# weibohuang0314/pixel_aware_gyro_aided_klt_feature_tracker

Measured on AMD Instinct MI355X. Metric: tracked features/sec (21x21, 3-lvl, 30 iter), higher is better.
Workload: dtype f32 sampling, f64 normal equations; 1 GPU; cfg1_euroc_752x480: 752x480 pair, 1000 keypoints (1000/GPU), gyro-predicted affine init, h=10, L=3, I=30 (synthetic stand-in for BASELINE configs[1]); mode=shard-weak, features_total=1000, features_active=1000, step_mode=graph

## Files before the change

__graft_entry__.py:

```python
from __future__ import annotations

import os
import subprocess
import sys

ROOT = os.path.dirname(os.path.abspath(__file__))
PKG = os.path.join(ROOT, "pixel_aware_gyro_aided_klt_feature_tracker_amd")
CSRC = os.path.join(PKG, "csrc")
HIP_LIB = os.path.join(PKG, "libpagk_hip.so")
HOST_LIB = os.path.join(PKG, "libpagk_tracker.so")

HIPCC_FLAGS = [
    "--offload-arch=gfx950", "-O3", "-std=c++17", "-fPIC", "-shared",
    "-ffp-contract=off", "-fno-fast-math",
    "-Wall", "-Wno-unused-function",
]


def _newer(target: str, sources: list[str]) -> bool:
    if not os.path.exists(target):
        return False
    t = os.path.getmtime(target)
    return all(os.path.getmtime(s) <= t for s in sources)

# ... 10 lines not shown

RESOURCE_CLAIMS = {
    "k_track_blockILi2ELi25ELi4ELb0ELb0ELb1": (128, 0, 4),
    "k_track_blockILi1ELi25ELi4ELb0ELb0ELb1": (96, 0, 4),
    "k_track_quadILi7ELb1": (128, 44, 4),
    "k_track_blockILi2ELi25ELi4ELb0ELb0ELb0": (128, 20, 4),
    "k_track_blockILi1ELi25ELi4ELb0ELb0ELb0": (128, 6, 4),
    "k_track_quadILi7ELb0": (128, 48, 4),
    "k_track_block_pyrILi2ELi25ELb0": (128, 24, 4),
    "k_track_resume_liveILi2ELi25ELb0": (128, 64, 4),
    "k_track_resumeILi2ELi25ELb0": (128, 64, 4),
    "k_track_resume_liveILi2ELi25ELb1": (128, 48, 4),
    "k_track_resumeILi2ELi25ELb1": (128, 48, 4),
    "k_track_block_pyrILi2ELi25ELb1": (128, 8, 4),
    "k_track_block5ILi2ELi25ELb1": (96, 16, 5),
    "k_rectifyILi1ELb1": (64, 0, 8),
    "k_rectifyILi3ELb1": (64, 0, 8),
    "k_rectifyILi4ELb1": (64, 0, 8),
    "k_match_choose": (64, 0, 8),
    "k_match_compact": (64, 0, 8),
    "k_radius_top2": (64, 0, 8),
    "k_klt_finish": (64, 0, 8),
    "k_pose_prep": (64, 0, 8),
    "k_pose_hyp": (176, 0, 2),
    "k_pose_recover": (112, 0, 4),
    "k_pose_gather": (64, 0, 8),
}


RESOURCE_CLAIMS_ALL_VARIANTS = {
# ... 208 lines not shown
```

include/pagk.h:

```cpp
#ifndef PAGK_H
#define PAGK_H

#include <stddef.h>
#include <stdint.h>

#ifdef __cplusplus
extern "C" {
#endif

#define PAGK_VERSION 303

#define PAGK_MAX_PYRAMIDS 8
#define PAGK_MAX_HALF_PATCH 15

enum {
    PAGK_OK = 0,
    PAGK_E_ARG = -1,
    PAGK_E_HIP = -2,
    PAGK_E_NOMEM = -3,
    PAGK_E_UNSUPPORTED = -4,
    PAGK_E_NODEVICE = -5,
    PAGK_E_NCCL = -6,
    PAGK_E_CAPACITY = -7
};
// ... 83 lines not shown
int pagk_check_launch(pagk_ctx *ctx);
int pagk_set_stream(pagk_ctx *ctx, void *hip_stream);

int pagk_set_kernel(pagk_ctx *ctx, int32_t which);
int pagk_has_variant(int32_t which);
int pagk_last_variant(const pagk_ctx *ctx);

int pagk_last_handover(pagk_ctx *ctx);

int pagk_priority_threshold(pagk_ctx *ctx);

int pagk_prio_hint_threshold(pagk_ctx *ctx);
int pagk_prio_hint_reset(pagk_ctx *ctx);
int pagk_prio_hint_get(pagk_ctx *ctx, int32_t n, int32_t *hints);
int pagk_prio_hint_set(pagk_ctx *ctx, int32_t n, const int32_t *hints);

int pagk_set_concurrency(pagk_ctx *ctx, int32_t streams);

int pagk_last_kernel_ms(pagk_ctx *ctx, float *track_ms, float *pyramid_ms);

int pagk_gyro_predict_device(pagk_ctx *ctx, const pagk_params *params, int32_t width, int32_t height,
                             const float *KRKinv, const float *r3, int32_t n, const float *d_pt_ref_un,
                             float *d_pt_predict_un, float *d_pt_predict, uint8_t *d_status, float *d_affine);
int pagk_gyro_predict_device_rot(pagk_ctx *ctx, const pagk_params *params, int32_t width, int32_t height,
                                 const float *d_rot, int32_t n, const float *d_pt_ref_un, float *d_pt_predict_un,
                                 float *d_pt_predict, uint8_t *d_status, float *d_affine);

int pagk_post_filter(int32_t n, int32_t half_patch, const uint8_t *status_pm,
                     const double *pix_err, const double *dist_pred, const float *pt_pm,
                     const float *pt_pm_un, uint8_t *status_out, float *pt_predict,
// ... 296 lines not shown
```

pixel_aware_gyro_aided_klt_feature_tracker_amd/capi.py:

```python
from __future__ import annotations

import ctypes as C
import os

import numpy as np

PKG_DIR = os.path.dirname(os.path.abspath(__file__))
LIB_PATH = os.environ.get("PAGK_LIB") or os.path.join(PKG_DIR, "libpagk_hip.so")

PAGK_OK = 0
PAGK_E_ARG = -1
PAGK_E_HIP = -2
PAGK_E_NOMEM = -3
PAGK_E_UNSUPPORTED = -4
PAGK_E_NODEVICE = -5
PAGK_E_NCCL = -6
PAGK_E_CAPACITY = -7


class Image(C.Structure):
    _fields_ = [("data", C.c_void_p), ("width", C.c_int32), ("height", C.c_int32), ("step", C.c_int64)]


class Params(C.Structure):
# ... 365 lines not shown
    lib.pagk_ncc_free.argtypes = [vp, _P(Image), _P(Image), i32, i32, vp, vp, vp, vp]
    if hasattr(lib, "pagk_selftest_divide"):
        lib.pagk_selftest_divide.restype = C.c_int
        lib.pagk_selftest_divide.argtypes = [vp, i32, vp, vp, vp, vp, vp, vp]
        lib.pagk_selftest_solve.restype = C.c_int
        lib.pagk_selftest_solve.argtypes = [vp, i32, vp, vp, C.c_uint32, vp, vp, vp, vp]
    if hasattr(lib, "pagk_prio_hint_reset"):
        lib.pagk_prio_hint_threshold.restype = C.c_int
        lib.pagk_prio_hint_threshold.argtypes = [vp]
        lib.pagk_prio_hint_reset.restype = C.c_int
        lib.pagk_prio_hint_reset.argtypes = [vp]
        lib.pagk_prio_hint_get.restype = C.c_int
        lib.pagk_prio_hint_get.argtypes = [vp, i32, vp]
        lib.pagk_prio_hint_set.restype = C.c_int
        lib.pagk_prio_hint_set.argtypes = [vp, i32, vp]
    if hasattr(lib, "pagk_priority_threshold"):
        lib.pagk_priority_threshold.restype = C.c_int
        lib.pagk_priority_threshold.argtypes = [vp]
    if hasattr(lib, "pagk_check_launch"):
        lib.pagk_check_launch.restype = C.c_int
        lib.pagk_check_launch.argtypes = [vp]
    if hasattr(lib, "pagk_selftest_repeat_sum"):
        lib.pagk_selftest_repeat_sum.restype = C.c_int
        lib.pagk_selftest_repeat_sum.argtypes = [vp, i32, vp, i32, vp, vp]
    if hasattr(lib, "pagk_selftest_sample"):
        lib.pagk_selftest_sample.restype = C.c_int
        lib.pagk_selftest_sample.argtypes = [vp, i32, i32, i32, i32, vp, vp]
    lib.pagk_match_features.restype = C.c_int
    lib.pagk_match_features.argtypes = [i32, i32, vp, vp, vp, vp, i32, vp, vp, vp, vp]
    lib.pagk_multi_create.restype = C.c_int
# ... 28 lines not shown
EXPORTED_SYMBOLS = [
    "pagk_version", "pagk_strerror", "pagk_last_error", "pagk_params_default", "pagk_inv_log_max_dist",
    "pagk_create", "pagk_destroy", "pagk_track", "pagk_track_pyr", "pagk_frame_upload", "pagk_frame_upload_pinned",
    "pagk_frame_set_device", "pagk_frame_download_level", "pagk_track_device", "pagk_track_device_fused", "pagk_sync",
    "pagk_set_stream", "pagk_set_kernel", "pagk_last_variant", "pagk_set_concurrency", "pagk_last_handover", "pagk_last_kernel_ms", "pagk_post_filter", "pagk_gyro_predict_device",
    "pagk_gyro_predict_device_rot",
    "pagk_geometry_scores_device", "pagk_geometry_scores", "pagk_geometry_select", "pagk_geometry_validation",
    "pagk_graph_begin", "pagk_graph_end", "pagk_graph_launch", "pagk_graph_destroy",
    "pagk_near_neighbors_device", "pagk_find_near_neighbors", "pagk_ncc_free", "pagk_match_features",
    "pagk_multi_create", "pagk_multi_unique_id", "pagk_multi_create_rank", "pagk_multi_destroy", "pagk_multi_world",
    "pagk_multi_local", "pagk_multi_ctx", "pagk_multi_last_error", "pagk_shard_range", "pagk_shard_layout",
    "pagk_multi_allgather", "pagk_track_sharded", "pagk_selftest_divide", "pagk_selftest_solve",
    "pagk_selftest_repeat_sum", "pagk_check_launch", "pagk_track_device_batch", "pagk_frame_set_device_batch", "pagk_priority_threshold",
    "pagk_multi_comm_count", "pagk_has_variant",
    "pagk_prio_hint_threshold", "pagk_prio_hint_reset", "pagk_prio_hint_get", "pagk_prio_hint_set",
    "pagk_fit_params_default", "pagk_geometry_fit_device", "pagk_geometry_fit", "pagk_geometry_validation_device",
    "pagk_geometry_validation_fit", "pagk_selftest_fit_samples",
    "pagk_pose_params_default", "pagk_pose_params_check", "pagk_pose_2d2d_device", "pagk_pose_from_matches_device",
    "pagk_pose_2d2d",
    "pagk_post_filter_device", "pagk_gyro_predict_device_live", "pagk_frame_handover_device", "pagk_frame_handover",
    "pagk_detect_params_default", "pagk_detect_corners_device", "pagk_detect_corners",
    "pagk_frame_handover_detect_device", "pagk_frame_handover_detect", "pagk_selftest_corner_response",
    "pagk_fast_params_default", "pagk_fast_params_check", "pagk_detect_fast_bounds", "pagk_detect_fast_device",
    "pagk_detect_fast", "pagk_frame_handover_fast_device", "pagk_frame_handover_fast", "pagk_selftest_fast_cells",
    "pagk_rectify_params_default", "pagk_rectify_params_check", "pagk_rectify_set_maps", "pagk_frame_rectify_device",
    "pagk_frame_rectify_pinned", "pagk_rectify", "pagk_undistort_maps",
    "pagk_orb_params_default", "pagk_orb_params_check", "pagk_orb_pattern_check", "pagk_orb_set_pattern",
    "pagk_orb_describe_device", "pagk_orb_describe", "pagk_orb_match_device", "pagk_orb_match",
    "pagk_selftest_sample",
    "pagk_lk_params_default", "pagk_lk_params_check", "pagk_lk_levels", "pagk_lk_pyramid_device", "pagk_lk_track_device",
# ... 939 lines not shown
        return int(self.lib.pagk_prio_hint_threshold(self.h))

    def prio_hint_reset(self):
        if hasattr(self.lib, "pagk_prio_hint_reset"):
            self._check(self.lib.pagk_prio_hint_reset(self.h), "pagk_prio_hint_reset")

    def prio_hint_get(self, n: int) -> np.ndarray:
        out = np.zeros(max(n, 0), np.int32)
        self._check(self.lib.pagk_prio_hint_get(self.h, n, out.ctypes.data_as(C.c_void_p)), "pagk_prio_hint_get")
        return out

    def prio_hint_set(self, hints) -> None:
        h = np.ascontiguousarray(hints, np.int32)
        self._check(self.lib.pagk_prio_hint_set(self.h, int(h.shape[0]), h.ctypes.data_as(C.c_void_p)), "pagk_prio_hint_set")

    def last_variant(self) -> int:
        return int(self.lib.pagk_last_variant(self.h))

    def last_handover(self) -> int:
        rc = int(self.lib.pagk_last_handover(self.h))
        if rc < 0:
            self._check(rc, "pagk_last_handover")
        return rc

    def set_concurrency(self, streams: int):
        self._check(self.lib.pagk_set_concurrency(self.h, streams), "pagk_set_concurrency")

    def last_kernel_ms(self):
        t, p = C.c_float(0), C.c_float(0)
        self._check(self.lib.pagk_last_kernel_ms(self.h, C.byref(t), C.byref(p)), "pagk_last_kernel_ms")
# ... 128 lines not shown
```

pixel_aware_gyro_aided_klt_feature_tracker_amd/csrc/pagk_device.h:

```cpp
#pragma once
#include <hip/hip_runtime.h>
#include <stdint.h>

namespace pagk {

constexpr int kMaxLevels = 8;

struct DevLevel {
    const uint32_t *quad;
    int cols, rows;
    float fcols, frows;
    float fcols_m1, frows_m1;
};

__device__ __forceinline__ int ld_agent(const int *p) { return __hip_atomic_load(p, __ATOMIC_RELAXED, __HIP_MEMORY_SCOPE_AGENT); }
__device__ __forceinline__ void st_agent(int *p, int v) { __hip_atomic_store(p, v, __ATOMIC_RELAXED, __HIP_MEMORY_SCOPE_AGENT); }

struct SuspState {
    int level;
    int iter;
    float dx, dy, dg, db, lastCost;
    int iters;
};

// ... 46 lines not shown
    int half, iterations;
    int prio_k;
    unsigned long long *prio_stats;
    const int *prio_kbuf;
    const int *prio_hint_in;
    int *prio_hint_out;
    int prio_hint_t;
    int has_gyro, illum, use_affine, penalty, calc_ncc;
    uint32_t solver;
    float lam_invlog;
    float lam_invlog_alpha;
    float alpha;
    double win_size_inv;
    int distort_on;
    float fx, fy, cx, cy, fx_inv, fy_inv, k1, k2, p1, p2, k3;
};

__device__ __forceinline__ DevLevel pin_level(const DevLevel &src) { return src; }

struct Coord {
    int i;
    float f;
    float omf;
};

template <bool CLAMP>
__device__ __forceinline__ Coord prep_coord(float x, float fmax, float fmax_m1)
{
    if (CLAMP) {
        x = fmaxf(x, 0.0f);
// ... 667 lines not shown
```

pixel_aware_gyro_aided_klt_feature_tracker_amd/csrc/pagk_hip.hip:

```cpp
#include <hip/hip_runtime.h>

#include <algorithm>
#include <array>
#include <cmath>
#include <cstdio>
#include <cstdlib>
#include <cstring>
#include <new>
#include <utility>
#include <vector>

#include "../../include/pagk.h"
#include "pagk_kernels.h"
#include "pagk_associate_kernel.h"
#include "pagk_pose_kernel.h"
#include "pagk_layout.h"
#include "pagk_select.h"
#include "pagk_prio_env.h"

using namespace pagk;

namespace {

constexpr int kSlots = 6;
constexpr int kUserSlots = 4;

struct DevBuf {
    void *ptr = nullptr;
    size_t bytes = 0;
    void *host = nullptr;
    bool mirrored = false;
};

// ... 27 lines not shown
        FAST,
        RECT_ENTRIES,
        RECT_STAGE,
        ORB_PATTERN,
        ORB_BLUR,
        ORB_KEYS,
        LK_PYR,
        LK_PYR_LAST = LK_PYR + kSlots - 1,
        ASSOC,
        POSE,
        POSEIO,
        QUAD_WS,
        SUSP,
        LV,
        PRIO_HINT,
        kBufs
    };
    DevBuf buf[kBufs];
    int fit_n = 0, fit_iters = 0;
    int pose_n = 0, pose_iters = 0;
    int rect_w = 0, rect_h = 0, rect_wp = 0;
    bool orb_pattern_set = false;
    struct LkPyr { int w = 0, h = 0, top = -1; } lk_pyr[kSlots];
    void *queue = nullptr;
    int quad_capacity[PAGK_MAX_HALF_PATCH + 1] = {};
    int rows_capacity[PAGK_MAX_HALF_PATCH + 1] = {};
    int rows_waves_cap = 0;
    int *susp_count_dev = nullptr;
    struct BatchDesc {
        void *host = nullptr, *dev = nullptr;
// ... 34 lines not shown
    std::vector<BatchDesc> graph_batch[kGraphs];
    std::vector<GraphSeg> cap_segs;
    hipEvent_t ev_trk[2] = {}, ev_pyr[2] = {};
    bool trk_timed = false, pyr_timed = false;
    int kernel = 0;
    bool last_handover = false;
    int concurrency = 1;
    int last_variant = -1;
    int mfma_min_features = 0x7fffffff;
    int wave_min_features = 6000;
    int quad_min_features = 7000;
    int block5_min_features = 2500;
    int prio_k = 4;
    unsigned long long *prio_stats = nullptr;
    int prio_hint_t = kPrioHintDefault;
    bool block5_window = true;
    int levels_min_features = 6000;
    int levels_shift = 0;
    bool levels_shared = false;
    bool unfused_pyramid = false;
    char err[256] = {0};
};

namespace {

#define HIPCHK(ctx, call)                                                                              \
    do {                                                                                               \
        hipError_t e_ = (call);                                                                        \
        if (e_ != hipSuccess) {                                                                        \
            snprintf((ctx)->err, sizeof((ctx)->err), "%s:%d %s -> %s", __FILE__, __LINE__, #call,     \
// ... 116 lines not shown
    Layout<N> lay_;
    void *base_ = nullptr, *own_ = nullptr;
    bool pending_ = false;
};

int capture_split(pagk_ctx *ctx)
{
    hipGraph_t g = nullptr;
    HIPCHK(ctx, hipStreamEndCapture(ctx->stream, &g));
    if (g) {
        pagk_ctx::GraphSeg seg;
        hipError_t e = hipGraphInstantiate(&seg.ex, g, nullptr, nullptr, 0);
        if (e != hipSuccess) {
            (void)hipGraphDestroy(g);
            ctx->capturing = false;
            snprintf(ctx->err, sizeof(ctx->err), "hipGraphInstantiate (segment) -> %s", hipGetErrorString(e));
            return PAGK_E_HIP;
        }
        seg.g = g;
        ctx->cap_segs.push_back(seg);
    }
    hipError_t e = hipStreamBeginCapture(ctx->stream, hipStreamCaptureModeThreadLocal);
    if (e != hipSuccess) {
        ctx->capturing = false;
        snprintf(ctx->err, sizeof(ctx->err), "hipStreamBeginCapture (next segment) -> %s", hipGetErrorString(e));
        return PAGK_E_HIP;
    }
    return PAGK_OK;
}
void destroy_segs(std::vector<pagk_ctx::GraphSeg> &v)
{
    for (auto &sg : v) {
        if (sg.ex) (void)hipGraphExecDestroy(sg.ex);
        if (sg.g) (void)hipGraphDestroy(sg.g);
    }
    v.clear();
}

int batch_desc_alloc(pagk_ctx *ctx, pagk_ctx::BatchDesc &d)
// ... 70 lines not shown
    for (int l = 0; l < L; l++) {
        s.u8[l] = lay.at<uint8_t>(s.block.ptr, l);
        s.quad[l] = lay.at<uint32_t>(s.block.ptr, L + l);
    }
    s.w = lw[0];
    s.h = lh[0];
    s.L = L;
    return PAGK_OK;
}

int slot_reserve(pagk_ctx *ctx, FrameSlot &s, int w, int h, int L)
{
    int lw[kMaxLevels], lh[kMaxLevels];
    int rc = level_dims(w, h, L, lw, lh);
    return rc ? rc : slot_alloc(ctx, s, lw, lh, L, NOT_IN_CAPTURE);
}

int make_pyr_args(const FrameSlot &s, const uint8_t *src0, int64_t pitch0, int wrap0, PyrArgs *out)
{
    int lw[kMaxLevels], lh[kMaxLevels];
    level_dims(s.w, s.h, s.L, lw, lh);
    PyrArgs pa;
    memset(&pa, 0, sizeof pa);
    pa.src = src0;
    pa.pitch = pitch0;
    pa.wrap0 = wrap0;
    pa.n_levels = s.L;
    int nb = 0;
    for (int l = 0; l < 4; l++) {
        pa.first_block[l] = nb;
// ... 21 lines not shown
}

int slot_build(pagk_ctx *ctx, FrameSlot &s, const uint8_t *src0, int64_t pitch0, int wrap0)
{
    s.pad0 = wrap0 ? 0 : 2;
    s.img0 = src0, s.pitch0 = pitch0;
    int lw[kMaxLevels], lh[kMaxLevels];
    level_dims(s.w, s.h, s.L, lw, lh);
    dim3 blk(32, 8);
    if (ctx->ev_pyr[0] && !in_capture(ctx)) HIPCHK(ctx, hipEventRecord(ctx->ev_pyr[0], ctx->stream));
    bool all_even = true;
    for (int l = 0; l + 1 < s.L; l++) all_even = all_even && !(lw[l] & 1) && !(lh[l] & 1);
    if (s.L <= 4 && !ctx->unfused_pyramid && all_even) {
        PyrArgs pa;
        const int nb = make_pyr_args(s, src0, pitch0, wrap0, &pa);
        hipLaunchKernelGGL(k_pyramid_fused, dim3(nb), dim3(256), 0, ctx->stream, pa);
        HIPCHK(ctx, hipGetLastError());
        if (ctx->ev_pyr[1] && !in_capture(ctx)) HIPCHK(ctx, hipEventRecord(ctx->ev_pyr[1], ctx->stream));
        if (!in_capture(ctx)) ctx->pyr_timed = true;
        s.wrap0 = wrap0;
        s.valid = true;
        return PAGK_OK;
    }
    const uint8_t *src = src0;
    int64_t pitch = pitch0;
    for (int l = 0; l < s.L; l++) {
        if (l > 0) {
            dim3 grd((lw[l] + 31) / 32, (lh[l] + 7) / 8);
            if (!(lw[l - 1] & 1) && !(lh[l - 1] & 1))
                hipLaunchKernelGGL(k_pyr_down, grd, blk, 0, ctx->stream, src, pitch, lw[l], lh[l], s.u8[l]);
            else
                hipLaunchKernelGGL(k_pyr_down_linear, grd, blk, 0, ctx->stream, src, pitch, lw[l - 1], lh[l - 1], lw[l],
// ... 307 lines not shown
    }
    const bool five = lean && k.block5 && select_block5(n, ctx->block5_min_features, ctx->block5_window, ctx->cus);
    const TrackFn kern = five ? k.block5 : k.block[lean];
    if (lds > 48 * 1024) {
        static thread_local bool configured[PAGK_MAX_HALF_PATCH + 1][2][16] = {};
        bool &done = configured[a.half][lean][ctx->device & 15];
        if (!done) {
            HIPCHK(ctx, hipFuncSetAttribute(reinterpret_cast<const void *>(kern), hipFuncAttributeMaxDynamicSharedMemorySize, (int)lds));
            done = true;
        }
    }
    HIPCHK(ctx, launch(kern, n, kBlock, lds, ctx->stream, a));
    return PAGK_OK;
}

int prio_hint_attach(pagk_ctx *ctx, int n, TrackArgs *a)
{
    DevBuf &hb = ctx->buf[pagk_ctx::PRIO_HINT];
    const size_t need = (size_t)n * sizeof(int32_t);
    if (need > hb.bytes) {
        if (in_capture(ctx)) return PAGK_OK;
        for (int k = 0; k < pagk_ctx::kGraphs; k++)
            if (ctx->graph_execs[k]) return PAGK_OK;
        if (int rc = reserve(ctx, hb, need, NOT_IN_CAPTURE_NOR_UNDER_GRAPH, "the priority hints", kLargestLaunchFirst)) return rc;
        HIPCHK(ctx, hipMemsetAsync(hb.ptr, 0, hb.bytes, ctx->stream));
    }
    a->prio_hint_in = a->prio_hint_out = static_cast<int *>(hb.ptr);
    return PAGK_OK;
}

int prio_hint_clear(pagk_ctx *ctx)
{
    DevBuf &hb = ctx->buf[pagk_ctx::PRIO_HINT];
    if (hb.ptr) HIPCHK(ctx, hipMemsetAsync(hb.ptr, 0, hb.bytes, ctx->stream));
    return PAGK_OK;
}

int launch_track(pagk_ctx *ctx, const pagk_params *p, const FrameSlot &sr, const FrameSlot &sc, int n,
                 const float *d_pt_ref, const float *d_pt_init, const float *d_affine, const uint8_t *d_status,
                 const pagk_outputs *o, const PyrArgs *pyr = nullptr, int pyr_blocks = 0, bool *pyr_done = nullptr,
                 bool hinted = true)
{
    if (pyr_done) *pyr_done = false;
    TrackArgs a;
    memset(&a, 0, sizeof a);
    a.n_levels = p->pyramids;
    for (int l = 0; l < p->pyramids; l++) {
        fill_level(a.l1[l], sr, l);
        fill_level(a.l2[l], sc, l);
// ... 27 lines not shown
        const bool lean = !a.penalty && a.solver == 0;
        const TrackKernels &k = track_kernels_of(a.half);
        const int variant = ctx->last_variant = select_variant(select_in(ctx, p, n));
        int rc = PAGK_OK;
        hipError_t e = hipSuccess;
        switch (variant) {
            case 1: e = launch(k_track_thread, (n + 63) / 64, 64, 0, ctx->stream, a); break;
            case 2: e = launch(k.mfma[lean], n, 128, track_mfma_lds_bytes(a.half), ctx->stream, a); break;
            case 3: e = launch(k.wave[lean], n, 64, track_wave_lds_bytes(a.half), ctx->stream, a); break;
            case 4: e = launch(k.relaxed, n, kBlock, track_block_lds_bytes(a.half), ctx->stream, a); break;
            case 5:
            case 7: rc = launch_quad(ctx, p, k, lean, variant == 7, n, a); break;
            case 6: rc = launch_rows(ctx, k, n, a); break;
            default:
                if (hinted && (rc = prio_hint_attach(ctx, n, &a))) break;
                rc = launch_block(ctx, k, lean, n, a, pyr, pyr_blocks, pyr_done);
                break;
        }
        if (rc) return rc;
        HIPCHK(ctx, e);
        HIPCHK(ctx, hipGetLastError());
    }
    if (ctx->ev_trk[1] && !in_capture(ctx)) HIPCHK(ctx, hipEventRecord(ctx->ev_trk[1], ctx->stream));
    if (!in_capture(ctx)) ctx->trk_timed = true;
    return PAGK_OK;
}

struct FeatPtrs {
    float *pt_ref, *pt_init, *affine;
    uint8_t *status_in;
    pagk_outputs out;
// ... 182 lines not shown
    if (getenv("PAGK_QUAD_MIN")) ctx->quad_min_features = atoi(getenv("PAGK_QUAD_MIN"));
    if (getenv("PAGK_BLOCK5_MIN")) ctx->block5_min_features = atoi(getenv("PAGK_BLOCK5_MIN")), ctx->block5_window = false;
    if (getenv("PAGK_LEVELS_MIN")) ctx->levels_min_features = atoi(getenv("PAGK_LEVELS_MIN"));
    if (getenv("PAGK_PRIO_K") && strcmp(getenv("PAGK_PRIO_K"), "auto") == 0) {
        struct { unsigned long long st[2]; int k, pad; } seed = {{3500ull, 1000ull}, ctx->prio_k, 0};
        if (hipMalloc(reinterpret_cast<void **>(&ctx->prio_stats), sizeof seed) != hipSuccess ||
            hipMemcpy(ctx->prio_stats, &seed, sizeof seed, hipMemcpyHostToDevice) != hipSuccess) {
            if (ctx->prio_stats) (void)hipFree(ctx->prio_stats);
            ctx->prio_stats = nullptr;
            (void)hipGetLastError();
        }
    } else if (getenv("PAGK_PRIO_K")) {
        ctx->prio_k = atoi(getenv("PAGK_PRIO_K")) < 0 ? 0 : atoi(getenv("PAGK_PRIO_K"));
    }
    if (getenv("PAGK_PRIO_HINT")) ctx->prio_hint_t = prio_hint_parse(getenv("PAGK_PRIO_HINT"), ctx->prio_hint_t);
    if (getenv("PAGK_LEVELS_XCD_SHIFT")) ctx->levels_shift = atoi(getenv("PAGK_LEVELS_XCD_SHIFT")) & 7;
    if (getenv("PAGK_LEVELS_SHARED")) ctx->levels_shared = atoi(getenv("PAGK_LEVELS_SHARED")) != 0;
    if (getenv("PAGK_QUAD_BUDGET")) ctx->quad_budget = atoi(getenv("PAGK_QUAD_BUDGET"));
    if (getenv("PAGK_ROWS_WAVES")) ctx->rows_waves_cap = atoi(getenv("PAGK_ROWS_WAVES"));
    if (getenv("PAGK_FINISHER_WGS")) ctx->finisher_wgs = atoi(getenv("PAGK_FINISHER_WGS"));
    if (getenv("PAGK_SUSPEND_LONE")) ctx->susp_lone = atoi(getenv("PAGK_SUSPEND_LONE"));
    if (getenv("PAGK_FINISHER_POLLS")) ctx->finisher_polls = atoi(getenv("PAGK_FINISHER_POLLS"));
    if (getenv("PAGK_LEVEL_POLLS")) ctx->level_polls = atoi(getenv("PAGK_LEVEL_POLLS"));
    if (hipStreamCreateWithFlags(&ctx->aux_stream, hipStreamNonBlocking) != hipSuccess ||
        hipEventCreateWithFlags(&ctx->ev_fork, hipEventDisableTiming) != hipSuccess ||
        hipEventCreateWithFlags(&ctx->ev_join, hipEventDisableTiming) != hipSuccess ||
        hipEventCreateWithFlags(&ctx->ev_batch, hipEventDisableTiming) != hipSuccess) {
        pagk_destroy(ctx);
        return PAGK_E_HIP;
    }
// ... 99 lines not shown
    if (!ctx) return PAGK_E_ARG;
    HIPCHK(ctx, hipSetDevice(ctx->device));
    return prio_hint_clear(ctx);
}

int pagk_prio_hint_get(pagk_ctx *ctx, int32_t n, int32_t *hints)
{
    if (!ctx || n < 0 || (n > 0 && !hints)) return PAGK_E_ARG;
    NOT_WHILE_CAPTURING(ctx, "pagk_prio_hint_get");
    HIPCHK(ctx, hipSetDevice(ctx->device));
    const DevBuf &hb = ctx->buf[pagk_ctx::PRIO_HINT];
    const size_t have = hb.bytes / sizeof(int32_t) < (size_t)n ? hb.bytes / sizeof(int32_t) : (size_t)n;
    memset(hints, 0, (size_t)n * sizeof(int32_t));
    if (have) HIPCHK(ctx, hipMemcpyAsync(hints, hb.ptr, have * sizeof(int32_t), hipMemcpyDeviceToHost, ctx->stream));
    HIPCHK(ctx, hipStreamSynchronize(ctx->stream));
    return PAGK_OK;
}

int pagk_prio_hint_set(pagk_ctx *ctx, int32_t n, const int32_t *hints)
{
    if (!ctx || n < 0 || (n > 0 && !hints)) return PAGK_E_ARG;
    NOT_WHILE_CAPTURING(ctx, "pagk_prio_hint_set");
    HIPCHK(ctx, hipSetDevice(ctx->device));
    DevBuf &hb = ctx->buf[pagk_ctx::PRIO_HINT];
    if (int rc = reserve(ctx, hb, (size_t)n * sizeof(int32_t), NOT_IN_CAPTURE_NOR_UNDER_GRAPH, "the priority hints", kLargestLaunchFirst)) return rc;
    if (int rc = prio_hint_clear(ctx)) return rc;
    if (n) HIPCHK(ctx, hipMemcpyAsync(hb.ptr, hints, (size_t)n * sizeof(int32_t), hipMemcpyHostToDevice, ctx->stream));
    HIPCHK(ctx, hipStreamSynchronize(ctx->stream));
    return PAGK_OK;
}

int pagk_check_launch(pagk_ctx *ctx)
{
    if (!ctx) return PAGK_E_ARG;
    return lv_check(ctx);
}

int pagk_set_concurrency(pagk_ctx *ctx, int32_t streams)
{
    if (!ctx || streams < 1 || streams > 64) return PAGK_E_ARG;
    ctx->concurrency = streams;
    return PAGK_OK;
}

int pagk_sync(pagk_ctx *ctx)
{
    if (!ctx) return PAGK_E_ARG;
    NOT_WHILE_CAPTURING(ctx, "pagk_sync");
    HIPCHK(ctx, hipStreamSynchronize(ctx->stream));
    return lv_check(ctx);
}

int pagk_last_kernel_ms(pagk_ctx *ctx, float *track_ms, float *pyramid_ms)
{
    if (!ctx) return PAGK_E_ARG;
    NOT_WHILE_CAPTURING(ctx, "pagk_last_kernel_ms");
    if (track_ms) {
        *track_ms = 0.0f;
        if (ctx->trk_timed) {
            HIPCHK(ctx, hipEventSynchronize(ctx->ev_trk[1]));
            HIPCHK(ctx, hipEventElapsedTime(track_ms, ctx->ev_trk[0], ctx->ev_trk[1]));
        }
    }
    if (pyramid_ms) {
// ... 1789 lines not shown
        for (auto &d : ctx->cap_batch)
            if (int ar = batch_desc_alloc(ctx, d)) {
                batch_desc_free(ctx->cap_batch);
                return ar;
            }
    }
    HIPCHK(ctx, hipStreamBeginCapture(ctx->stream, hipStreamCaptureModeThreadLocal));
    ctx->capturing = true;
    return PAGK_OK;
}

int pagk_graph_end(pagk_ctx *ctx, int32_t *graph_id)
{
    if (!ctx || !ctx->capturing || !graph_id) return PAGK_E_ARG;
    ctx->capturing = false;
    hipGraph_t g = nullptr;
    HIPCHK(ctx, hipStreamEndCapture(ctx->stream, &g));
    int id = -1;
    for (int k = 0; k < pagk_ctx::kGraphs; k++)
        if (!ctx->graph_execs[k]) {
            id = k;
            break;
        }
    if (id < 0 || !g) {
        if (g) (void)hipGraphDestroy(g);
        destroy_segs(ctx->cap_segs);
        batch_desc_free(ctx->cap_batch);
        snprintf(ctx->err, sizeof(ctx->err), id < 0 ? "all %d graph slots are in use" : "capture produced no graph (%d)", pagk_ctx::kGraphs);
        return PAGK_E_ARG;
    }
    hipGraphExec_t ex = nullptr;
    hipError_t e = hipGraphInstantiate(&ex, g, nullptr, nullptr, 0);
    if (e != hipSuccess) {
        (void)hipGraphDestroy(g);
        destroy_segs(ctx->cap_segs);
        batch_desc_free(ctx->cap_batch);
        snprintf(ctx->err, sizeof(ctx->err), "hipGraphInstantiate -> %s", hipGetErrorString(e));
        return PAGK_E_HIP;
    }
    ctx->graphs[id] = g;
    ctx->graph_execs[id] = ex;
    ctx->pre_segs[id] = std::move(ctx->cap_segs);
    ctx->cap_segs.clear();
    batch_desc_free(ctx->graph_batch[id]);
    ctx->graph_batch[id] = std::move(ctx->cap_batch);
    ctx->cap_batch.clear();
    ctx->cap_batch_used = 0;
    *graph_id = id;
    return PAGK_OK;
}

int pagk_graph_launch(pagk_ctx *ctx, int32_t graph_id)
{
    if (!ctx || ctx->capturing || graph_id < 0 || graph_id >= pagk_ctx::kGraphs || !ctx->graph_execs[graph_id]) return PAGK_E_ARG;
    for (pagk_ctx::GraphSeg &sg : ctx->pre_segs[graph_id]) {
        if (sg.kind == pagk_ctx::GraphSeg::GRAPH) {
            HIPCHK(ctx, hipGraphLaunch(sg.ex, ctx->stream));
        } else if (sg.kind == pagk_ctx::GraphSeg::FINISHER) {
            HIPCHK(ctx, hipEventRecord(ctx->ev_fork, ctx->stream));
            HIPCHK(ctx, hipStreamWaitEvent(ctx->aux_stream, ctx->ev_fork, 0));
            void *kargs[] = {&sg.args};
            HIPCHK(ctx, hipLaunchKernel(sg.fn, dim3(sg.grid), dim3(kBlock), kargs, sg.lds, ctx->aux_stream));
            HIPCHK(ctx, hipEventRecord(ctx->ev_join, ctx->aux_stream));
        } else {
            HIPCHK(ctx, hipStreamWaitEvent(ctx->stream, ctx->ev_join, 0));
        }
    }
    HIPCHK(ctx, hipGraphLaunch(ctx->graph_execs[graph_id], ctx->stream));
    return PAGK_OK;
}

int pagk_graph_destroy(pagk_ctx *ctx, int32_t graph_id)
{
    if (!ctx || graph_id < 0 || graph_id >= pagk_ctx::kGraphs || !ctx->graph_execs[graph_id]) return PAGK_E_ARG;
    HIPCHK(ctx, hipStreamSynchronize(ctx->stream));
    if (ctx->aux_stream) HIPCHK(ctx, hipStreamSynchronize(ctx->aux_stream));
    (void)hipGraphExecDestroy(ctx->graph_execs[graph_id]);
    (void)hipGraphDestroy(ctx->graphs[graph_id]);
    destroy_segs(ctx->pre_segs[graph_id]);
    batch_desc_free(ctx->graph_batch[graph_id]);
    ctx->graph_execs[graph_id] = nullptr;
    ctx->graphs[graph_id] = nullptr;
    return lv_check(ctx);
}

int pagk_geometry_scores_device(pagk_ctx *ctx, const double *H21, const double *H12, const double *F21,
                                int32_t n, const float *d_pts1, const float *d_pts2, float sigma,
                                uint8_t *d_inliers_H, uint8_t *d_inliers_F, float *d_scores)
{
    if (!ctx || !H21 || !H12 || !F21 || n < 0 || !d_scores) return PAGK_E_ARG;
    if (n > 0 && (!d_pts1 || !d_pts2 || !d_inliers_H || !d_inliers_F)) return PAGK_E_ARG;
    HIPCHK(ctx, hipSetDevice(ctx->device));
    ScoreArgs a;
    memset(&a, 0, sizeof a);
    for (int k = 0; k < 9; k++) a.H21[k] = H21[k], a.H12[k] = H12[k], a.F21[k] = F21[k];
    a.pts1 = d_pts1, a.pts2 = d_pts2, a.n = n, a.sigma = sigma;
    a.inl_H = d_inliers_H, a.inl_F = d_inliers_F, a.scores = d_scores;
// ... 952 lines not shown
```

pixel_aware_gyro_aided_klt_feature_tracker_amd/csrc/pagk_kernels.h:

```cpp
#pragma once
#include <type_traits>
#include "pagk_device.h"
#include "pagk_chain_asm.h"
#include "pagk_prio.h"

namespace pagk {

__global__ void k_pyr_down(const uint8_t *__restrict__ src, int64_t pitch, int dw, int dh,
                           uint8_t *__restrict__ dst)
{
    int x = blockIdx.x * blockDim.x + threadIdx.x;
    int y = blockIdx.y * blockDim.y + threadIdx.y;
    if (x >= dw || y >= dh) return;
    const uint8_t *r0 = src + (int64_t)(2 * y) * pitch + 2 * x;
    const uint8_t *r1 = r0 + pitch;
    dst[(int64_t)y * dw + x] = (uint8_t)((r0[0] + r0[1] + r1[0] + r1[1] + 2) >> 2);
}

__global__ void k_pyr_down_linear(const uint8_t *__restrict__ src, int64_t pitch, int w, int h, int dw, int dh,
                                  double scale_x, double scale_y, uint8_t *__restrict__ dst)
{
    const int dx = blockIdx.x * blockDim.x + threadIdx.x;
    const int dy = blockIdx.y * blockDim.y + threadIdx.y;
    if (dx >= dw || dy >= dh) return;
// ... 92 lines not shown
}

__device__ __forceinline__ void pyr_block(const PyrArgs &a, int b, int tid)
{
    if (b < a.first_block[1]) {
        pyr_emit<0>(a, (b - a.first_block[0]) * 256 + tid);
    } else if (b < a.first_block[2]) {
        pyr_emit<1>(a, (b - a.first_block[1]) * 256 + tid);
    } else if (b < a.first_block[3]) {
        pyr_emit<2>(a, (b - a.first_block[2]) * 256 + tid);
    } else if (b < a.first_block[4]) {
        pyr_emit<3>(a, (b - a.first_block[3]) * 256 + tid);
    }
}

__global__ void __launch_bounds__(256) k_pyramid_fused(PyrArgs a)
{
    pyr_block(a, (int)blockIdx.x, (int)threadIdx.x);
}

struct PyrBatchEntry {
    PyrArgs a;
    int block_base, pad_;
};
__global__ void __launch_bounds__(256) k_pyramid_fused_batch(const PyrBatchEntry *__restrict__ frames, int k)
{
    int f = 0;
    for (int j = 1; j < k; j++) f = (int)blockIdx.x >= frames[j].block_base ? j : f;
    pyr_block(frames[f].a, (int)blockIdx.x - frames[f].block_base, (int)threadIdx.x);
}

struct PredictArgs {
    int n, width, height;
// ... 838 lines not shown
        for (int k = 0; k < 6; k++) dbgp[(size_t)i * 16 + k] = st[k];
        dbgp[(size_t)i * 16 + 6] = (unsigned long long)iters;
        dbgp[(size_t)i * 16 + 7] = rt_begin;
        for (int k = 8; k < 11; k++) dbgp[(size_t)i * 16 + k] = st[k];
        dbgp[(size_t)i * 16 + 11] = __builtin_amdgcn_s_memrealtime();
        dbgp[(size_t)i * 16 + 12] = st[12];
        dbgp[(size_t)i * 16 + 13] = st[13];
    }
#endif
#undef STAMP
}

template <int NR, int TAIL, int WAVES = 4, bool MFMA = false, bool RELAXED = false, bool LEAN = false>
__global__ void __launch_bounds__(WAVES * 64, 4) k_track_block(TrackArgs a)
{
    track_block_body<NR, TAIL, WAVES, MFMA, RELAXED, LEAN>(a, (int)blockIdx.x);
}

template <int NR, int TAIL, bool LEAN = false>
__global__ void __launch_bounds__(256, 5) k_track_block5(TrackArgs a)
{
    track_block_body<NR, TAIL, 4, false, false, LEAN, false>(a, (int)blockIdx.x);
}

__device__ __forceinline__ SuspState load_susp_state(const TrackArgs &a, int i)
{
    const int *p = reinterpret_cast<const int *>(&a.susp_state[i]);
    SuspState st;
    st.level = ld_agent(p + 0), st.iter = ld_agent(p + 1);
    st.dx = __int_as_float(ld_agent(p + 2)), st.dy = __int_as_float(ld_agent(p + 3));
    st.dg = __int_as_float(ld_agent(p + 4)), st.db = __int_as_float(ld_agent(p + 5));
    st.lastCost = __int_as_float(ld_agent(p + 6)), st.iters = ld_agent(p + 7);
    return st;
}

template <int NR, int TAIL, bool LEAN = false>
__global__ void __launch_bounds__(256, 4) k_track_resume_live(TrackArgs a)
// ... 39 lines not shown
        if (entry <= 0) continue;
        const int i = entry - 1;
        const SuspState st = load_susp_state(a, i);
        track_block_body<NR, TAIL, 4, false, false, LEAN>(a, i, &st);
        __syncthreads();
    }
}

template <int NR, int TAIL, bool LEAN = false>
__global__ void __launch_bounds__(256, 4) k_track_block_pyr(TrackArgs a, PyrArgs pa)
{
    if ((int)blockIdx.x >= a.n) {
        pyr_block(pa, (int)blockIdx.x - a.n, (int)threadIdx.x);
        return;
    }
    track_block_body<NR, TAIL, 4, false, false, LEAN>(a, (int)blockIdx.x);
}

}

#include "pagk_wave_kernel.h"
#include "pagk_quad_kernel.h"
#ifdef PAGK_ALL_VARIANTS
#include "pagk_rows_kernel.h"
#endif
#include "pagk_score_kernel.h"
#include "pagk_fit_kernel.h"
#include "pagk_handover_kernel.h"
#include "pagk_detect_kernel.h"
#include "pagk_fast_kernel.h"
#include "pagk_rectify_kernel.h"
// ... 5 lines not shown
```

pixel_aware_gyro_aided_klt_feature_tracker_amd/csrc/pagk_prio.h:

```cpp
#pragma once

#ifndef PAGK_PRIO_MODE
#define PAGK_PRIO_MODE 1
#endif

namespace pagk {
__device__ __forceinline__ void prio_account(const TrackArgs &a, int i, int iters, int levels)
{
    if (a.prio_stats && (i & 7) == 0) {
        __hip_atomic_fetch_add(a.prio_stats + 0, (unsigned long long)iters, __ATOMIC_RELAXED, __HIP_MEMORY_SCOPE_AGENT);
        __hip_atomic_fetch_add(a.prio_stats + 1, (unsigned long long)levels, __ATOMIC_RELAXED, __HIP_MEMORY_SCOPE_AGENT);
        if ((i & 63) == 0 && iters <= 4 * levels) {
            const unsigned long long it = __hip_atomic_load(a.prio_stats + 0, __ATOMIC_RELAXED, __HIP_MEMORY_SCOPE_AGENT);
            const unsigned long long lv = __hip_atomic_load(a.prio_stats + 1, __ATOMIC_RELAXED, __HIP_MEMORY_SCOPE_AGENT);
            if (lv > 0) {
                int k = (int)ceilf((float)it / (float)lv);
                k = k < 3 ? 3 : (k > 12 ? 12 : k);
                __hip_atomic_store(const_cast<int *>(a.prio_kbuf), k, __ATOMIC_RELAXED, __HIP_MEMORY_SCOPE_AGENT);
            }
        }
    }
}

constexpr int kPrioBoost = 1 << 20;
__device__ __forceinline__ void prio_hint_store(const TrackArgs &a, int i, int iters)
{
    if (a.prio_hint_out) a.prio_hint_out[i] = iters;
}
}
#if PAGK_PRIO_MODE == 0
#define PAGK_PRIO_DECL(hinted)
#define PAGK_PRIO_TIER
#define PAGK_PRIO_RESET
#define PRIO(n) __builtin_amdgcn_s_setprio(n);
#define PAGK_PRIO_N_CHAIN 3
#define PAGK_PRIO_N_SAMP 2
#define PAGK_PRIO_N_COST 1
#define PAGK_PRIO_N_REST 0
#else
#define PAGK_PRIO_DECL(hinted)                                                                                       \
    int tier_now = 0;                                                                                                \
    const int prio_kv = !kPrioByWork ? 0 : (a.prio_kbuf ? __builtin_amdgcn_readfirstlane(*a.prio_kbuf) : a.prio_k);  \
// ... 32 lines not shown
```

Baseline: 12.69 million features/s.

## Dispatch features longest-first using iteration hints sorted inside pyramid kernel

Adds a counting sort of per-feature iteration hints from the previous frame. It runs as an extra lead block in the fused pyramid kernel and writes a dispatch-order array. The track kernels then map blockIdx through that array, so features expected to need the most iterations are scheduled first, which is meant to cut tail imbalance at the end of the grid. In exchange it adds an indirection load per block, an extra block and LDS in the pyramid launch, and fairly intricate host-side state tracking for graph capture and replay, including a device sync when a graph is replayed on a different stream.

```diff
diff --git a/__graft_entry__.py b/__graft_entry__.py
--- a/__graft_entry__.py
+++ b/__graft_entry__.py
@@ -48,6 +48,7 @@
     "k_track_resumeILi2ELi25ELb1": (128, 48, 4),
     "k_track_block_pyrILi2ELi25ELb1": (128, 8, 4),
     "k_track_block5ILi2ELi25ELb1": (96, 16, 5),
+    "k_pyramid_fused": (64, 0, 8),
     "k_rectifyILi1ELb1": (64, 0, 8),
     "k_rectifyILi3ELb1": (64, 0, 8),
     "k_rectifyILi4ELb1": (64, 0, 8),
diff --git a/include/pagk.h b/include/pagk.h
--- a/include/pagk.h
+++ b/include/pagk.h
@@ -121,6 +121,9 @@
 int pagk_prio_hint_reset(pagk_ctx *ctx);
 int pagk_prio_hint_get(pagk_ctx *ctx, int32_t n, int32_t *hints);
 int pagk_prio_hint_set(pagk_ctx *ctx, int32_t n, const int32_t *hints);
+
+int pagk_dispatch_order_enabled(pagk_ctx *ctx);
+int pagk_dispatch_order_get(pagk_ctx *ctx, int32_t n, int32_t *order, int32_t *in_force);
 
 int pagk_set_concurrency(pagk_ctx *ctx, int32_t streams);
 
diff --git a/pixel_aware_gyro_aided_klt_feature_tracker_amd/capi.py b/pixel_aware_gyro_aided_klt_feature_tracker_amd/capi.py
--- a/pixel_aware_gyro_aided_klt_feature_tracker_amd/capi.py
+++ b/pixel_aware_gyro_aided_klt_feature_tracker_amd/capi.py
@@ -403,6 +403,11 @@
         lib.pagk_prio_hint_get.argtypes = [vp, i32, vp]
         lib.pagk_prio_hint_set.restype = C.c_int
         lib.pagk_prio_hint_set.argtypes = [vp, i32, vp]
+    if hasattr(lib, "pagk_dispatch_order_get"):
+        lib.pagk_dispatch_order_enabled.restype = C.c_int
+        lib.pagk_dispatch_order_enabled.argtypes = [vp]
+        lib.pagk_dispatch_order_get.restype = C.c_int
+        lib.pagk_dispatch_order_get.argtypes = [vp, i32, vp, vp]
     if hasattr(lib, "pagk_priority_threshold"):
         lib.pagk_priority_threshold.restype = C.c_int
         lib.pagk_priority_threshold.argtypes = [vp]
@@ -461,6 +466,7 @@
     "pagk_selftest_repeat_sum", "pagk_check_launch", "pagk_track_device_batch", "pagk_frame_set_device_batch", "pagk_priority_threshold",
     "pagk_multi_comm_count", "pagk_has_variant",
     "pagk_prio_hint_threshold", "pagk_prio_hint_reset", "pagk_prio_hint_get", "pagk_prio_hint_set",
+    "pagk_dispatch_order_enabled", "pagk_dispatch_order_get",
     "pagk_fit_params_default", "pagk_geometry_fit_device", "pagk_geometry_fit", "pagk_geometry_validation_device",
     "pagk_geometry_validation_fit", "pagk_selftest_fit_samples",
     "pagk_pose_params_default", "pagk_pose_params_check", "pagk_pose_2d2d_device", "pagk_pose_from_matches_device",
@@ -1430,6 +1436,16 @@
         h = np.ascontiguousarray(hints, np.int32)
         self._check(self.lib.pagk_prio_hint_set(self.h, int(h.shape[0]), h.ctypes.data_as(C.c_void_p)), "pagk_prio_hint_set")
 
+    def dispatch_order_enabled(self) -> bool:
+        return bool(self.lib.pagk_dispatch_order_enabled(self.h))
+
+    def dispatch_order_get(self, n: int):
+        out = np.zeros(max(n, 0), np.int32)
+        in_force = C.c_int32(0)
+        self._check(self.lib.pagk_dispatch_order_get(self.h, n, out.ctypes.data_as(C.c_void_p), C.byref(in_force)),
+                    "pagk_dispatch_order_get")
+        return out, bool(in_force.value)
+
     def last_variant(self) -> int:
         return int(self.lib.pagk_last_variant(self.h))
 
diff --git a/pixel_aware_gyro_aided_klt_feature_tracker_amd/csrc/pagk_device.h b/pixel_aware_gyro_aided_klt_feature_tracker_amd/csrc/pagk_device.h
--- a/pixel_aware_gyro_aided_klt_feature_tracker_amd/csrc/pagk_device.h
+++ b/pixel_aware_gyro_aided_klt_feature_tracker_amd/csrc/pagk_device.h
@@ -84,6 +84,7 @@
     double win_size_inv;
     int distort_on;
     float fx, fy, cx, cy, fx_inv, fy_inv, k1, k2, p1, p2, k3;
+    const int *order;
 };
 
 __device__ __forceinline__ DevLevel pin_level(const DevLevel &src) { return src; }
diff --git a/pixel_aware_gyro_aided_klt_feature_tracker_amd/csrc/pagk_hip.hip b/pixel_aware_gyro_aided_klt_feature_tracker_amd/csrc/pagk_hip.hip
--- a/pixel_aware_gyro_aided_klt_feature_tracker_amd/csrc/pagk_hip.hip
+++ b/pixel_aware_gyro_aided_klt_feature_tracker_amd/csrc/pagk_hip.hip
@@ -17,6 +17,7 @@
 #include "pagk_layout.h"
 #include "pagk_select.h"
 #include "pagk_prio_env.h"
+#include "pagk_order.h"
 
 using namespace pagk;
 
@@ -74,6 +75,7 @@
         SUSP,
         LV,
         PRIO_HINT,
+        DISPATCH_ORDER,
         kBufs
     };
     DevBuf buf[kBufs];
@@ -138,6 +140,8 @@
     int prio_k = 4;
     unsigned long long *prio_stats = nullptr;
     int prio_hint_t = kPrioHintDefault;
+    bool graph_order[kGraphs] = {};
+    OrderState order;
     bool block5_window = true;
     int levels_min_features = 6000;
     int levels_shift = 0;
@@ -284,6 +288,7 @@
         if (e != hipSuccess) {
             (void)hipGraphDestroy(g);
             ctx->capturing = false;
+            (void)ctx->order.capture_ended();
             snprintf(ctx->err, sizeof(ctx->err), "hipGraphInstantiate (segment) -> %s", hipGetErrorString(e));
             return PAGK_E_HIP;
         }
@@ -293,6 +298,7 @@
     hipError_t e = hipStreamBeginCapture(ctx->stream, hipStreamCaptureModeThreadLocal);
     if (e != hipSuccess) {
         ctx->capturing = false;
+        (void)ctx->order.capture_ended();
         snprintf(ctx->err, sizeof(ctx->err), "hipStreamBeginCapture (next segment) -> %s", hipGetErrorString(e));
         return PAGK_E_HIP;
     }
@@ -393,6 +399,15 @@
     int lw[kMaxLevels], lh[kMaxLevels];
     int rc = level_dims(w, h, L, lw, lh);
     return rc ? rc : slot_alloc(ctx, s, lw, lh, L, NOT_IN_CAPTURE);
+}
+
+int capture_kind(pagk_ctx *ctx) { return ctx->capturing ? 1 : (in_capture(ctx) ? 2 : 0); }
+
+OrderArgs order_build_args(pagk_ctx *ctx)
+{
+    const DevBuf &hb = ctx->buf[pagk_ctx::PRIO_HINT], &ob = ctx->buf[pagk_ctx::DISPATCH_ORDER];
+    const int n = ctx->order.build_n(ctx->stream, ctx->cus, (long long)(hb.bytes / sizeof(int32_t)), (long long)(ob.bytes / sizeof(int32_t)), capture_kind(ctx));
+    return {static_cast<const int *>(hb.ptr), static_cast<int *>(ob.ptr), n};
 }
 
 int make_pyr_args(const FrameSlot &s, const uint8_t *src0, int64_t pitch0, int wrap0, PyrArgs *out)
@@ -444,8 +459,10 @@
     if (s.L <= 4 && !ctx->unfused_pyramid && all_even) {
         PyrArgs pa;
         const int nb = make_pyr_args(s, src0, pitch0, wrap0, &pa);
-        hipLaunchKernelGGL(k_pyramid_fused, dim3(nb), dim3(256), 0, ctx->stream, pa);
+        const OrderArgs oa = order_build_args(ctx);
+        hipLaunchKernelGGL(k_pyramid_fused, dim3(nb + (oa.n > 0 ? 1 : 0)), dim3(256), order_lds_bytes(oa.n), ctx->stream, pa, oa);
         HIPCHK(ctx, hipGetLastError());
+        if (oa.n > 0) ctx->order.built(oa.n, ctx->stream, capture_kind(ctx));
         if (ctx->ev_pyr[1] && !in_capture(ctx)) HIPCHK(ctx, hipEventRecord(ctx->ev_pyr[1], ctx->stream));
         if (!in_capture(ctx)) ctx->pyr_timed = true;
         s.wrap0 = wrap0;
@@ -783,10 +800,21 @@
     return PAGK_OK;
 }
 
+int order_reserve(pagk_ctx *ctx, int n)
+{
+    DevBuf &ob = ctx->buf[pagk_ctx::DISPATCH_ORDER];
+    if (!ctx->order.on || !order_serves(n, ctx->cus) || (size_t)n * sizeof(int32_t) <= ob.bytes || in_capture(ctx)) return PAGK_OK;
+    for (int k = 0; k < pagk_ctx::kGraphs; k++)
+        if (ctx->graph_execs[k]) return PAGK_OK;
+    ctx->order.array_replaced();
+    return reserve(ctx, ob, (size_t)n * sizeof(int32_t), NOT_IN_CAPTURE_NOR_UNDER_GRAPH, "the dispatch order", kLargestLaunchFirst);
+}
+
 int prio_hint_attach(pagk_ctx *ctx, int n, TrackArgs *a)
 {
     DevBuf &hb = ctx->buf[pagk_ctx::PRIO_HINT];
     const size_t need = (size_t)n * sizeof(int32_t);
+    if (int rc = order_reserve(ctx, n)) return rc;
     if (need > hb.bytes) {
         if (in_capture(ctx)) return PAGK_OK;
         for (int k = 0; k < pagk_ctx::kGraphs; k++)
@@ -802,6 +830,7 @@
 {
     DevBuf &hb = ctx->buf[pagk_ctx::PRIO_HINT];
     if (hb.ptr) HIPCHK(ctx, hipMemsetAsync(hb.ptr, 0, hb.bytes, ctx->stream));
+    ctx->order.hints_cleared();
     return PAGK_OK;
 }
 
@@ -859,7 +888,11 @@
             case 6: rc = launch_rows(ctx, k, n, a); break;
             default:
                 if (hinted && (rc = prio_hint_attach(ctx, n, &a))) break;
+                if (a.prio_hint_in && ctx->order.usable(n, ctx->stream, ctx->cus, capture_kind(ctx)) &&
+                    ctx->buf[pagk_ctx::DISPATCH_ORDER].bytes >= (size_t)n * sizeof(int32_t))
+                    a.order = static_cast<const int *>(ctx->buf[pagk_ctx::DISPATCH_ORDER].ptr);
                 rc = launch_block(ctx, k, lean, n, a, pyr, pyr_blocks, pyr_done);
+                if (!rc && hinted) ctx->order.launched(a.prio_hint_out ? n : 0, ctx->stream, a.order != nullptr, capture_kind(ctx));
                 break;
         }
         if (rc) return rc;
@@ -1072,6 +1105,7 @@
         ctx->prio_k = atoi(getenv("PAGK_PRIO_K")) < 0 ? 0 : atoi(getenv("PAGK_PRIO_K"));
     }
     if (getenv("PAGK_PRIO_HINT")) ctx->prio_hint_t = prio_hint_parse(getenv("PAGK_PRIO_HINT"), ctx->prio_hint_t);
+    if (getenv("PAGK_DISPATCH_ORDER")) ctx->order.on = atoi(getenv("PAGK_DISPATCH_ORDER")) != 0;
     if (getenv("PAGK_LEVELS_XCD_SHIFT")) ctx->levels_shift = atoi(getenv("PAGK_LEVELS_XCD_SHIFT")) & 7;
     if (getenv("PAGK_LEVELS_SHARED")) ctx->levels_shared = atoi(getenv("PAGK_LEVELS_SHARED")) != 0;
     if (getenv("PAGK_QUAD_BUDGET")) ctx->quad_budget = atoi(getenv("PAGK_QUAD_BUDGET"));
@@ -1201,6 +1235,24 @@
     memset(hints, 0, (size_t)n * sizeof(int32_t));
     if (have) HIPCHK(ctx, hipMemcpyAsync(hints, hb.ptr, have * sizeof(int32_t), hipMemcpyDeviceToHost, ctx->stream));
     HIPCHK(ctx, hipStreamSynchronize(ctx->stream));
+    ctx->order.stream_idle(ctx->stream);
+    return PAGK_OK;
+}
+
+int pagk_dispatch_order_enabled(pagk_ctx *ctx) { return ctx ? (ctx->order.on ? 1 : 0) : PAGK_E_ARG; }
+
+int pagk_dispatch_order_get(pagk_ctx *ctx, int32_t n, int32_t *order, int32_t *in_force)
+{
+    if (!ctx || n < 0 || (n > 0 && !order)) return PAGK_E_ARG;
+    NOT_WHILE_CAPTURING(ctx, "pagk_dispatch_order_get");
+    HIPCHK(ctx, hipSetDevice(ctx->device));
+    const DevBuf &ob = ctx->buf[pagk_ctx::DISPATCH_ORDER];
+    const size_t have = ob.bytes / sizeof(int32_t) < (size_t)n ? ob.bytes / sizeof(int32_t) : (size_t)n;
+    for (int32_t i = 0; i < n; i++) order[i] = i;
+    if (have) HIPCHK(ctx, hipMemcpyAsync(order, ob.ptr, have * sizeof(int32_t), hipMemcpyDeviceToHost, ctx->stream));
+    HIPCHK(ctx, hipStreamSynchronize(ctx->stream));
+    ctx->order.stream_idle(ctx->stream);
+    if (in_force) *in_force = (have == (size_t)n && ctx->order.usable(n, ctx->stream, ctx->cus, 0)) ? 1 : 0;
     return PAGK_OK;
 }
 
@@ -1214,6 +1266,9 @@
     if (int rc = prio_hint_clear(ctx)) return rc;
     if (n) HIPCHK(ctx, hipMemcpyAsync(hb.ptr, hints, (size_t)n * sizeof(int32_t), hipMemcpyHostToDevice, ctx->stream));
     HIPCHK(ctx, hipStreamSynchronize(ctx->stream));
+    if (int rc = order_reserve(ctx, n)) return rc;
+    ctx->order.stream_idle(ctx->stream);
+    ctx->order.hints_set(n);
     return PAGK_OK;
 }
 
@@ -1235,6 +1290,7 @@
     if (!ctx) return PAGK_E_ARG;
     NOT_WHILE_CAPTURING(ctx, "pagk_sync");
     HIPCHK(ctx, hipStreamSynchronize(ctx->stream));
+    ctx->order.stream_idle(ctx->stream);
     return lv_check(ctx);
 }
 
@@ -3054,6 +3110,7 @@
 {
     if (!ctx || !ctx->capturing || !graph_id) return PAGK_E_ARG;
     ctx->capturing = false;
+    const bool carries_order = ctx->order.capture_ended();
     hipGraph_t g = nullptr;
     HIPCHK(ctx, hipStreamEndCapture(ctx->stream, &g));
     int id = -1;
@@ -3080,6 +3137,7 @@
     }
     ctx->graphs[id] = g;
     ctx->graph_execs[id] = ex;
+    ctx->graph_order[id] = carries_order;
     ctx->pre_segs[id] = std::move(ctx->cap_segs);
     ctx->cap_segs.clear();
     batch_desc_free(ctx->graph_batch[id]);
@@ -3093,6 +3151,7 @@
 int pagk_graph_launch(pagk_ctx *ctx, int32_t graph_id)
 {
     if (!ctx || ctx->capturing || graph_id < 0 || graph_id >= pagk_ctx::kGraphs || !ctx->graph_execs[graph_id]) return PAGK_E_ARG;
+    if (ctx->graph_order[graph_id] && ctx->order.replay(ctx->stream)) HIPCHK(ctx, hipDeviceSynchronize());
     for (pagk_ctx::GraphSeg &sg : ctx->pre_segs[graph_id]) {
         if (sg.kind == pagk_ctx::GraphSeg::GRAPH) {
             HIPCHK(ctx, hipGraphLaunch(sg.ex, ctx->stream));
@@ -3121,6 +3180,11 @@
     batch_desc_free(ctx->graph_batch[graph_id]);
     ctx->graph_execs[graph_id] = nullptr;
     ctx->graphs[graph_id] = nullptr;
+    ctx->graph_order[graph_id] = false;
+    ctx->order.stream_idle(ctx->stream);
+    bool alive = false;
+    for (int k = 0; k < pagk_ctx::kGraphs; k++) alive = alive || ctx->graph_execs[k];
+    if (!alive) ctx->order.graphs_gone();
     return lv_check(ctx);
 }
 
diff --git a/pixel_aware_gyro_aided_klt_feature_tracker_amd/csrc/pagk_kernels.h b/pixel_aware_gyro_aided_klt_feature_tracker_amd/csrc/pagk_kernels.h
--- a/pixel_aware_gyro_aided_klt_feature_tracker_amd/csrc/pagk_kernels.h
+++ b/pixel_aware_gyro_aided_klt_feature_tracker_amd/csrc/pagk_kernels.h
@@ -3,6 +3,7 @@
 #include "pagk_device.h"
 #include "pagk_chain_asm.h"
 #include "pagk_prio.h"
+#include "pagk_order.h"
 
 namespace pagk {
 
@@ -130,9 +131,83 @@
     }
 }
 
-__global__ void __launch_bounds__(256) k_pyramid_fused(PyrArgs a)
-{
-    pyr_block(a, (int)blockIdx.x, (int)threadIdx.x);
+struct OrderArgs {
+    const int *hints;
+    int *order;
+    int n;
+};
+
+__device__ __forceinline__ void order_block(const OrderArgs &o, int tid)
+{
+    extern __shared__ __attribute__((aligned(16))) unsigned char order_lds[];
+    int (*s_at)[kOrderClasses] = reinterpret_cast<int (*)[kOrderClasses]>(order_lds);
+    uint8_t *s_class = order_lds + 4 * kOrderClasses * sizeof(int);
+    const int n = o.n < kOrderMaxN ? o.n : kOrderMaxN;
+    const int wave = tid >> 6, lane = tid & 63;
+    const int quarter = ((n + 255) >> 8) << 6;
+    const int lo = wave * quarter, hi = lo + quarter < n ? lo + quarter : n;
+    for (int k = tid; k < 4 * kOrderClasses; k += 256) (&s_at[0][0])[k] = 0;
+    __syncthreads();
+    for (int i = lo + lane; i < hi; i += 64) {
+        const int c = kOrderKeyMax - order_key(o.hints[i]);
+        s_class[i] = (uint8_t)c;
+        atomicAdd(&s_at[wave][c], 1);
+    }
+    __syncthreads();
+    if (wave == 0) {
+        static_assert(kOrderClasses == 128, "two classes per lane of one wave");
+        int cnt[2][4], pair = 0;
+#pragma unroll
+        for (int k = 0; k < 2; k++)
+#pragma unroll
+            for (int w = 0; w < 4; w++) pair += cnt[k][w] = s_at[w][2 * lane + k];
+        int incl = pair;
+#pragma unroll
+        for (int d = 1; d < 64; d <<= 1) {
+            const int up = __shfl_up(incl, d);
+            incl += lane >= d ? up : 0;
+        }
+        int at = incl - pair;
+#pragma unroll
+        for (int k = 0; k < 2; k++)
+#pragma unroll
+            for (int w = 0; w < 4; w++) {
+                s_at[w][2 * lane + k] = at;
+                at += cnt[k][w];
+            }
+    }
+    __syncthreads();
+    for (int base = lo; base < hi; base += 64) {
+        const int i = base + lane;
+        const bool valid = i < hi;
+        const int c = valid ? (int)s_class[i] : 255;
+        unsigned long long same = ~0ull;
+#pragma unroll
+        for (int b = 0; b < 8; b++) {
+            const bool bit = (c >> b) & 1;
+            const unsigned long long with = __ballot(bit);
+            same &= bit ? with : ~with;
+        }
+        const int below = __popcll(same & ((1ull << lane) - 1ull)), all = __popcll(same);
+        int at = 0;
+        if (valid) {
+            at = s_at[wave][c];
+            o.order[at + below] = i;
+        }
+        __builtin_amdgcn_wave_barrier();
+        if (valid && below == all - 1) s_at[wave][c] = at + all;
+        __builtin_amdgcn_wave_barrier();
+    }
+}
+
+__global__ void __launch_bounds__(256) k_pyramid_fused(PyrArgs a, OrderArgs o)
+{
+    const int lead = o.n > 0 ? 1 : 0;
+    if (lead && blockIdx.x == 0) {
+        order_block(o, (int)threadIdx.x);
+        return;
+    }
+    pyr_block(a, (int)blockIdx.x - lead, (int)threadIdx.x);
 }
 
 struct PyrBatchEntry {
@@ -1001,13 +1076,16 @@
 template <int NR, int TAIL, int WAVES = 4, bool MFMA = false, bool RELAXED = false, bool LEAN = false>
 __global__ void __launch_bounds__(WAVES * 64, 4) k_track_block(TrackArgs a)
 {
-    track_block_body<NR, TAIL, WAVES, MFMA, RELAXED, LEAN>(a, (int)blockIdx.x);
+    if constexpr (MFMA || RELAXED)
+        track_block_body<NR, TAIL, WAVES, MFMA, RELAXED, LEAN>(a, (int)blockIdx.x);
+    else
+        track_block_body<NR, TAIL, WAVES, MFMA, RELAXED, LEAN>(a, dispatch_feature(a));
 }
 
 template <int NR, int TAIL, bool LEAN = false>
 __global__ void __launch_bounds__(256, 5) k_track_block5(TrackArgs a)
 {
-    track_block_body<NR, TAIL, 4, false, false, LEAN, false>(a, (int)blockIdx.x);
+    track_block_body<NR, TAIL, 4, false, false, LEAN, false>(a, dispatch_feature(a));
 }
 
 __device__ __forceinline__ SuspState load_susp_state(const TrackArgs &a, int i)
@@ -1077,7 +1155,7 @@
         pyr_block(pa, (int)blockIdx.x - a.n, (int)threadIdx.x);
         return;
     }
-    track_block_body<NR, TAIL, 4, false, false, LEAN>(a, (int)blockIdx.x);
+    track_block_body<NR, TAIL, 4, false, false, LEAN>(a, dispatch_feature(a));
 }
 
 }
diff --git a/pixel_aware_gyro_aided_klt_feature_tracker_amd/csrc/pagk_order.h b/pixel_aware_gyro_aided_klt_feature_tracker_amd/csrc/pagk_order.h
--- /dev/null
+++ b/pixel_aware_gyro_aided_klt_feature_tracker_amd/csrc/pagk_order.h
@@ -0,0 +1,86 @@
+#pragma once
+
+#include <cstdint>
+
+namespace pagk {
+
+constexpr int kOrderKeyMax = 127;
+constexpr int kOrderClasses = kOrderKeyMax + 1;
+constexpr int kOrderMaxN = 8192;
+
+constexpr int order_key(int32_t hint) { return hint < 0 ? 0 : (hint > kOrderKeyMax ? kOrderKeyMax : (int)hint); }
+
+inline void order_reference(int n, const int32_t *hints, int32_t *order)
+{
+    int start[kOrderClasses + 1] = {};
+    for (int i = 0; i < n; i++) start[kOrderKeyMax - order_key(hints[i]) + 1]++;
+    for (int c = 0; c < kOrderClasses; c++) start[c + 1] += start[c];
+    for (int i = 0; i < n; i++) order[start[kOrderKeyMax - order_key(hints[i])]++] = i;
+}
+
+constexpr unsigned order_lds_bytes(int n) { return n > 0 ? 4u * kOrderClasses * 4u + (((unsigned)n + 255u) & ~255u) : 0u; }
+
+constexpr bool order_serves(long long n, int cus) { return n > cus && n <= kOrderMaxN; }
+
+struct OrderState {
+    bool on = true;
+    int want_n = 0;
+    int built_n = 0;
+    const void *built_on = nullptr;
+    const void *home = nullptr;
+    int frozen_n = 0;
+    bool in_capture = false;
+
+    int build_n(const void *stream, int cus, long long hint_slots, long long order_slots, int capture) const
+    {
+        if (!on || capture == 2 || !order_serves(want_n, cus) || hint_slots < want_n || order_slots < want_n) return 0;
+        if (home && home != stream) return 0;
+        if (frozen_n && frozen_n != want_n) return 0;
+        return want_n;
+    }
+    void built(int n, const void *stream, int capture)
+    {
+        built_n = n;
+        built_on = stream;
+        touch(n, stream, capture);
+    }
+    bool usable(int n, const void *stream, int cus, int capture) const
+    {
+        return on && capture != 2 && order_serves(n, cus) && built_n == n && built_on == stream && (!home || home == stream) &&
+               (!frozen_n || frozen_n == n);
+    }
+    void launched(int n, const void *stream, bool used, int capture)
+    {
+        want_n = n;
+        built_n = 0;
+        if (used) touch(n, stream, capture);
+    }
+    bool capture_ended()
+    {
+        const bool carried = in_capture;
+        in_capture = false;
+        built_n = 0;
+        return carried;
+    }
+    bool replay(const void *stream)
+    {
+        const bool elsewhere = home && home != stream;
+        home = stream;
+        built_n = 0;
+        return elsewhere;
+    }
+    void hints_cleared() { built_n = want_n = 0; }
+    void hints_set(int n) { built_n = 0, want_n = n; }
+    void array_replaced() { built_n = 0; }
+    void stream_idle(const void *stream) { if (home == stream) home = nullptr; }
+    void graphs_gone() { frozen_n = 0; }
+
+private:
+    void touch(int n, const void *stream, int capture)
+    {
+        if (capture) frozen_n = n, in_capture = true;
+        else home = stream;
+    }
+};
+
+}
diff --git a/pixel_aware_gyro_aided_klt_feature_tracker_amd/csrc/pagk_prio.h b/pixel_aware_gyro_aided_klt_feature_tracker_amd/csrc/pagk_prio.h
--- a/pixel_aware_gyro_aided_klt_feature_tracker_amd/csrc/pagk_prio.h
+++ b/pixel_aware_gyro_aided_klt_feature_tracker_amd/csrc/pagk_prio.h
@@ -26,6 +26,12 @@
 __device__ __forceinline__ void prio_hint_store(const TrackArgs &a, int i, int iters)
 {
     if (a.prio_hint_out) a.prio_hint_out[i] = iters;
+}
+
+__device__ __forceinline__ int dispatch_feature(const TrackArgs &a)
+{
+    const int b = (int)blockIdx.x;
+    return a.order ? __builtin_amdgcn_readfirstlane(a.order[b]) : b;
 }
 }
 #if PAGK_PRIO_MODE == 0
```

Result: faster. 13.74 million features/s (median of 6 runs) (+8.3%).
